# HiromasaYamanishi/furusato_recommend

Hardware: AMD Instinct MI355X
Metric: BPR positive-edges/sec (LightGCN-3 d=64, 1000000 x 100000 / 20000000 edges) (higher is better)
Workload: dtype f32; 1 GPU; C2: LightGCN 3-layer d=64, synthetic 1000000 users x 100000 items / 20000000 edges (uniform); users=1000000, items=100000, edges=20000000, graph=uniform, dim=64, layers=3, bpr_batch_per_rank=2048, global_batch=2048, ranks=1, parallelism=dp1 (user-sharded, RCCL none gradient exchange)

## Files before the change

furusato_recommend_amd/_lib.py:

```python
from __future__ import annotations

import ctypes
import os
from ctypes import (POINTER, Structure, c_float, c_int, c_int32, c_int64,
                    c_size_t, c_uint64, c_void_p, c_char_p)

import torch

_HERE = os.path.dirname(os.path.abspath(__file__))
LIB_PATH = os.environ.get("MIREC_LIB") or os.path.join(_HERE, "libmirec.so")

MIREC_OK = 0
ERR_WORKSPACE = 4
ERR_RANGE = 5
IN_PRESCALED, IN_RAW, IN_SPARSE, IN_NONE = 0, 1, 2, 3
SUPPORTED_DIMS = (4, 8, 16, 32, 64, 128, 256)


class MirecError(RuntimeError):
    pass


class CSR(Structure):
    _fields_ = [
        ("rowptr", c_void_p), ("col", c_void_p), ("dinv", c_void_p),
        ("n_rows", c_int64), ("nnz", c_int64), ("split", c_int32),
        ("_pad", c_int32), ("n_long", c_int64), ("n_seg", c_int64),
        ("long_rows", c_void_p), ("long_segptr", c_void_p),
        ("seg_row", c_void_p), ("seg_beg", c_void_p),
        ("col_sorted", c_void_p), ("n_sorted", c_int64), ("val", c_void_p),
    ]


class AdamH(Structure):
    _fields_ = [
        ("one_minus_beta1", c_float), ("beta2", c_float),
        ("one_minus_beta2", c_float), ("neg_step_size", c_float),
        ("bc2_sqrt", c_float), ("eps", c_float),
    ]


class Prop(Structure):
    _fields_ = [
        ("dim", c_int32), ("in_mode", c_int32), ("x_in", c_void_p),
        ("slot", c_void_p), ("seed_in", c_void_p), ("seed", c_void_p),
        ("addend", c_void_p), ("seed2", c_void_p), ("divisor", c_float),
        ("_pad", c_float), ("out", c_void_p), ("xs_out", c_void_p),
        ("param", c_void_p), ("exp_avg", c_void_p), ("exp_avg_sq", c_void_p),
        ("adam", AdamH), ("partial", c_void_p), ("row_mask", c_void_p),
        ("in_mask", c_void_p), ("out_mask", c_void_p), ("row_list", c_void_p),
        ("row_count", c_void_p),
        ("row_list_cap", c_int64), ("narrow_max", c_int32), ("adam_stream", c_int32),
        ("wide_list", c_void_p), ("wide_count", c_void_p),
        ("scale_src", c_void_p), ("scale_dst", c_void_p), ("scale_next", c_void_p),
    ]


class Drop(Structure):
    _fields_ = [("keep_prob", c_float), ("transposed", c_int32), ("seed", c_uint64)]


class SeedBits(Structure):
    _fields_ = [("bits", c_void_p), ("split", c_int64), ("shift", c_int32 * 2),
                ("words", c_int32 * 2)]


class Sweep(Structure):
    _fields_ = [
        ("row0", c_int64), ("n_rows", c_int64), ("n_src", c_int64),
        ("tile_rows", c_int32), ("group_rows", c_int32), ("groups", c_int32),
        ("n_tiles", c_int32), ("band_rows", c_int32), ("_pad", c_int32),
        ("gptr", c_void_p), ("ent", c_void_p),
    ]


class SweepWave(Structure):
    _fields_ = [
        ("row0", c_int64), ("n_rows", c_int64), ("src0", c_int64), ("n_src", c_int64),
        ("n_slots", c_int64),
        ("tile_rows", c_int32), ("wave_rows", c_int32), ("n_tiles", c_int32),
# ... 438 lines not shown
```

furusato_recommend_amd/csrc/prop.hip:

```cpp
#include <mutex>
#include <set>
#include <type_traits>
#include <utility>

#include "common.h"

namespace mirec {

struct PropK {
  const int64_t *rowptr;
  const int32_t *col;
  const float *dinv;
  int64_t n_rows;
  int64_t n_seg;
  const int32_t *seg_row;
  const int64_t *seg_beg;
  int32_t split;
  const float *x_in;
  const int32_t *slot;
  const float *seed_in;
  const float *seed;
  const float *addend;
  const float *seed2;
  float divisor;
// ... 106 lines not shown
          v[u] = f4_zero();
      }
#pragma unroll
      for (int u = 0; u < UNROLL; ++u) {
        if (MODE != MIREC_IN_PRESCALED || WEIGHTED)
          acc = f4_fma(w[u], v[u], acc);
        else
          acc = f4_add(acc, v[u]);
      }
    }
  }
  if constexpr (DROPOUT) acc = f4_scale(a.drop_scale, acc);
  return acc;
}

template <int D>
__device__ __forceinline__ float4 combine_groups(float4 s) {
  constexpr int LPR = D / 4;
#pragma unroll
  for (int m = LPR; m < 64; m <<= 1) s = f4_add(s, f4_shfl_xor(s, m));
  return s;
}

typedef float f32x4_t __attribute__((ext_vector_type(4)));
__device__ __forceinline__ float4 ld4_nt(const float *p) {
  const f32x4_t v = __builtin_nontemporal_load(reinterpret_cast<const f32x4_t *>(p));
  return make_float4(v.x, v.y, v.z, v.w);
}
__device__ __forceinline__ void st4_nt(float *p, float4 v) {
  const f32x4_t t = {v.x, v.y, v.z, v.w};
  __builtin_nontemporal_store(t, reinterpret_cast<f32x4_t *>(p));
}

template <int D, bool SCALED = false, bool STREAM = false>
__device__ __forceinline__ void row_epilogue(const PropK &a, int64_t row, float4 s, int sub) {
  const float di = a.dinv[row];
  float dn = di;
  if (SCALED && a.xs_out != nullptr) dn = a.scale_next[row];
  const int64_t off = row * D + sub * 4;
  float4 z = f4_scale(di, s);
  int sl = -1;
  if (a.slot != nullptr && (a.seed != nullptr || a.seed2 != nullptr)) sl = a.slot[row];
  if (a.seed != nullptr && sl >= 0) z = f4_add(z, ld4(a.seed + (int64_t)sl * D + sub * 4));
  if (a.xs_out != nullptr && a.param == nullptr) st4(a.xs_out + off, f4_scale(dn, z));
  if (a.out == nullptr && a.param == nullptr) return;
  if (a.out_mask != nullptr && a.param == nullptr && a.out_mask[row] == 0) return;
  float4 o = z;
  if (a.addend != nullptr) o = f4_add(o, ld4(a.addend + off));
  if (a.divisor != 1.f) o = f4_div(o, a.divisor);
  if (a.seed2 != nullptr && sl >= 0) o = f4_add(o, ld4(a.seed2 + (int64_t)sl * D + sub * 4));
  if (a.param != nullptr) {
    float4 p, m, v;
    if constexpr (STREAM) {
      p = ld4_nt(a.param + off), m = ld4_nt(a.m + off), v = ld4_nt(a.v + off);
    } else {
      p = ld4(a.param + off), m = ld4(a.m + off), v = ld4(a.v + off);
    }
    adam1(p.x, m.x, v.x, o.x, a.adam);
    adam1(p.y, m.y, v.y, o.y, a.adam);
    adam1(p.z, m.z, v.z, o.z, a.adam);
    adam1(p.w, m.w, v.w, o.w, a.adam);
    if constexpr (STREAM) {
      st4_nt(a.param + off, p);
      st4_nt(a.m + off, m);
      st4_nt(a.v + off, v);
    } else {
      st4(a.param + off, p);
      st4(a.m + off, m);
      st4(a.v + off, v);
    }
    if (a.out != nullptr) st4(a.out + off, o);
    if (a.xs_out != nullptr) st4(a.xs_out + off, f4_scale(dn, p));
  } else {
    st4(a.out + off, o);
  }
}

constexpr int kWavesPerBlock = 4;

template <int D, int UNROLL, int MODE, bool MASKED, bool ROWMASK, bool WEIGHTED, bool SCALED,
          bool DROPOUT, bool STREAM = false>
__device__ __forceinline__ void prop_work(const PropK &a, int64_t w, int64_t nrows,
                                          int64_t row_waves) {
  constexpr int LPR = D / 4;
  constexpr int G = 64 / LPR;
  constexpr int NARROW_UNROLL = UNROLL < 4 ? 4 : UNROLL;
  const int lane = threadIdx.x & 63;
  const int sub = lane % LPR;
  const int grp = lane / LPR;
  if (w < row_waves) {
    const int64_t idx = w * G + grp;
    bool have = idx < nrows;
    int32_t row = 0;
    if (have) row = (ROWMASK && a.row_list != nullptr) ? a.row_list[idx] : (int32_t)idx;
    if (ROWMASK && have) have = bit_set(a.row_mask, row);
    int64_t beg = 0, end = 0;
    if (have) {
      beg = a.rowptr[row];
      end = a.rowptr[row + 1];
      if (a.split > 0 && end - beg > a.split) {
        have = false;
        beg = end = 0;
      }
    }
    const int64_t deg = have ? end - beg : 0;
    if (G > 1 && __ballot(deg > a.narrow_max) == 0ull) {
      float4 s = gather<D, NARROW_UNROLL, MODE, MASKED, WEIGHTED, true, SCALED, DROPOUT>(
          a, beg, end, lane, row);
      if (have) row_epilogue<D, SCALED, STREAM>(a, row, s, sub);
// ... 437 lines not shown
  int32_t n_tiles;
  int32_t band_rows;
  int32_t n_bands;
  int32_t row_bits;
};

constexpr int kAuxNone = 0, kAuxPace = 1, kAuxStamp = 2;
constexpr int kPaceLabels = 8;
constexpr int kPaceLineWords = 32;
constexpr int kPaceRegionWords = (2 * kPaceLabels + 1) * kPaceLineWords;
constexpr int kPaceMaxNaps = 8;
constexpr int kPaceMaxNapUnits = 16;
constexpr int kXccIdReg = 20 | (3 << 11);

struct SweepAuxK {
  unsigned *ws;
  int32_t lead;
  int32_t every;
  int32_t nap;
  long long *stamps;
  int32_t *meta;
};

__device__ __forceinline__ unsigned pace_read(const unsigned *p) {
  unsigned v;
  asm volatile("s_load_dword %0, %1, 0x0 glc\n\ts_waitcnt lgkmcnt(0)"
               : "=&s"(v)
               : "s"(p)
               : "memory");
  return v;
}

template <int D, int U, bool SCALED, int AUX = kAuxNone, bool PACKED = false,
          bool STREAM = false, bool INMASK = false>
__device__ __forceinline__ void sweep_wave_work(const PropK &a, const SweepWaveK &s,
                                                const SweepAuxK &x = SweepAuxK{}) {
  constexpr int LPR = D / 4;
  constexpr int G = 64 / LPR;
  constexpr int NB = 64 / (U * G);
  static_assert(G == 4 && U * G == MIREC_SWEEP_BATCH && kSweepThreads / 64 == MIREC_SWEEP_WAVES,
                "the host layout's steps, batches and waves");
  static_assert(!INMASK || (!SCALED && !STREAM && AUX != kAuxStamp && NB >= 3),
                "the masked forms a step uses");
  extern __shared__ float4 sweep_acc[];
  const int lane = threadIdx.x & 63;
  const int sub = lane % LPR;
  const int g = lane / LPR;
  const int wid = __builtin_amdgcn_readfirstlane(threadIdx.x >> 6);
  using Slot = typename std::conditional<PACKED, unsigned, long long>::type;
  const Slot *slots = reinterpret_cast<const Slot *>(s.slot);
  [[maybe_unused]] const int col_bits = 32 - s.row_bits;
  const Slot kPadRow = PACKED ? (Slot)(~0u << col_bits) : (Slot)0xffffffff00000000ull;
  const int64_t last = s.n_slots - 1;
  [[maybe_unused]] auto slot_col = [&](Slot v) -> int64_t {
    if constexpr (PACKED) return s.src0 + (int64_t)(v & ~kPadRow);
    return (int64_t)(v & 0xffffffffll);
  };
  int adv = 0, told = 0, due = 0;
  unsigned *pace_reg = nullptr, *pace_sum = nullptr;
  if constexpr (AUX == kAuxPace) {
    const int label = (int)__builtin_amdgcn_s_getreg(kXccIdReg) & (kPaceLabels - 1);
    pace_reg = x.ws + (2 * label) * kPaceLineWords;
    pace_sum = pace_reg + kPaceLineWords;
    due = x.every;
    if (wid == 0 && lane == 0)
      (void)__hip_atomic_fetch_add(pace_reg, 1u, __ATOMIC_RELAXED, __HIP_MEMORY_SCOPE_AGENT);
  }
  auto pace = [&]() {
    if constexpr (AUX == kAuxPace) {
      if (wid != 0) return;
      ++adv;
      if (--due != 0) return;
      due = x.every;
      if (lane == 0)
        (void)__hip_atomic_fetch_add(pace_sum, (unsigned)(adv - told), __ATOMIC_RELAXED,
                                     __HIP_MEMORY_SCOPE_AGENT);
// ... 79 lines not shown
#pragma unroll
        for (int u = 0; u < U; ++u) {
          const int src = k * U * G + u * G + g;
          const int j = __shfl(lcol, src);
          r[u] = __shfl(crow, src);
          v[u] = ld4(a.x_in + (int64_t)j * D + sub * 4);
        }
#pragma unroll
        for (int u = 0; u < U; ++u) {
          if (pr[u] >= 0) {
            float4 *p = &sweep_acc[pr[u] * LPR + sub];
            *p = f4_add(*p, pv[u]);
          }
        }
#pragma unroll
        for (int u = 0; u < U; ++u) {
          pv[u] = v[u];
          pr[u] = r[u];
        }
      }
      pos += 64;
      cur = nxt;
      if constexpr (INMASK) {
        asm volatile("" : "+v"(nmask));
        cmask = nmask;
      }
    }
    while (band + 1 < s.n_bands) {
      pace();
      __builtin_amdgcn_s_barrier();
      ++band;
      stamp(band);
    }
#pragma unroll
    for (int u = 0; u < U; ++u) {
      if (pr[u] >= 0) {
        float4 *p = &sweep_acc[pr[u] * LPR + sub];
        *p = f4_add(*p, pv[u]);
      }
    }
    for (int lr = lr0 + g; lr < lr1; lr += G)
      row_epilogue<D, SCALED, STREAM>(a, s.row0 + tile_row0 + lr, sweep_acc[lr * LPR + sub],
                                      sub);
    if constexpr (AUX == kAuxStamp) {
      stamp(s.n_bands);
      if (wid == 0) {
        long long *o = x.stamps + (int64_t)tile * (s.n_bands + 1);
        for (int b = lane; b <= s.n_bands; b += 64) o[b] = stamp_lds[b];
        if (lane == 0) {
          x.meta[2 * tile] = (int32_t)blockIdx.x;
          x.meta[2 * tile + 1] = (int32_t)__builtin_amdgcn_s_getreg(kXccIdReg);
        }
      }
    }
    __syncthreads();
  }
  if constexpr (AUX == kAuxPace) {
    if (wid == 0 && lane == 0) {
      (void)__hip_atomic_fetch_add(pace_sum, 0u - (unsigned)told, __ATOMIC_RELAXED,
                                   __HIP_MEMORY_SCOPE_AGENT);
      (void)__hip_atomic_fetch_add(pace_reg, 0u - 1u, __ATOMIC_RELAXED, __HIP_MEMORY_SCOPE_AGENT);
      asm volatile("s_waitcnt vmcnt(0)" ::: "memory");
      unsigned *done = x.ws + 2 * kPaceLabels * kPaceLineWords;
      const unsigned left = __hip_atomic_fetch_add(done, 1u, __ATOMIC_RELAXED,
                                                   __HIP_MEMORY_SCOPE_AGENT);
      if (left == gridDim.x - 1) {
        for (int i = 0; i <= 2 * kPaceLabels; ++i)
          __hip_atomic_store(x.ws + i * kPaceLineWords, 0u, __ATOMIC_RELAXED,
                             __HIP_MEMORY_SCOPE_AGENT);
      }
    }
  }
}

template <int D, int U, bool SCALED, bool PACKED = false, bool STREAM = false>
__global__ __launch_bounds__(kSweepThreads) __attribute__((amdgpu_waves_per_eu(4, 4)))
MIREC_NO_PK_F32 void prop_sweep_wave_kernel(PropK a, SweepWaveK s) {
  sweep_wave_work<D, U, SCALED, kAuxNone, PACKED, STREAM>(a, s);
}

template <int D, int U, bool SCALED, int AUX, bool PACKED = false, bool STREAM = false>
__global__ __launch_bounds__(kSweepThreads) __attribute__((amdgpu_waves_per_eu(4, 4)))
MIREC_NO_PK_F32 void prop_sweep_wave_aux_kernel(PropK a, SweepWaveK s, SweepAuxK x) {
  sweep_wave_work<D, U, SCALED, AUX, PACKED, STREAM>(a, s, x);
}

template <int D, int U, bool PACKED>
__global__ __launch_bounds__(kSweepThreads) __attribute__((amdgpu_waves_per_eu(4, 4)))
MIREC_NO_PK_F32 void prop_sweep_wave_masked_kernel(PropK a, SweepWaveK s) {
  sweep_wave_work<D, U, false, kAuxNone, PACKED, false, true>(a, s);
}

template <int D, int U, int AUX, bool PACKED>
__global__ __launch_bounds__(kSweepThreads) __attribute__((amdgpu_waves_per_eu(4, 4)))
MIREC_NO_PK_F32 void prop_sweep_wave_masked_aux_kernel(PropK a, SweepWaveK s, SweepAuxK x) {
  sweep_wave_work<D, U, false, AUX, PACKED, false, true>(a, s, x);
}

using PropFn = void (*)(PropK);

template <int D, int UNROLL>
static PropFn prop_kernel_for(int mode, bool masked, bool rowmask, bool weighted, bool scaled,
                              bool dropout) {
  if (mode == MIREC_IN_SPARSE) masked = true;
  if (mode == MIREC_IN_NONE) weighted = dropout = false;
#define MIREC_PROP_CASE(MODE_W, MASKED)                               \
  case (MODE_W) * 2 + (MASKED):                                       \
    return rowmask ? prop_kernel<D, UNROLL, (MODE_W), MASKED, true>   \
                   : prop_kernel<D, UNROLL, (MODE_W), MASKED, false>;
  switch ((mode | (weighted ? kWeighted : 0) | (scaled ? kScaled : 0) |
           (dropout ? kDropout : 0)) * 2 + masked) {
    MIREC_PROP_CASE(MIREC_IN_PRESCALED | kWeighted, false)
    MIREC_PROP_CASE(MIREC_IN_PRESCALED, false)
    MIREC_PROP_CASE(MIREC_IN_PRESCALED | kWeighted, true)
    MIREC_PROP_CASE(MIREC_IN_PRESCALED, true)
    MIREC_PROP_CASE(MIREC_IN_RAW | kWeighted, false)
    MIREC_PROP_CASE(MIREC_IN_RAW, false)
    MIREC_PROP_CASE(MIREC_IN_RAW | kWeighted, true)
    MIREC_PROP_CASE(MIREC_IN_RAW, true)
    MIREC_PROP_CASE(MIREC_IN_SPARSE | kWeighted, true)
    MIREC_PROP_CASE(MIREC_IN_SPARSE, true)
    MIREC_PROP_CASE(MIREC_IN_PRESCALED | kScaled, false)
    MIREC_PROP_CASE(MIREC_IN_PRESCALED | kScaled, true)
    MIREC_PROP_CASE(MIREC_IN_RAW | kScaled, false)
    MIREC_PROP_CASE(MIREC_IN_RAW | kScaled, true)
    MIREC_PROP_CASE(MIREC_IN_SPARSE | kScaled, true)
    MIREC_PROP_CASE(MIREC_IN_NONE | kScaled, false)
    MIREC_PROP_CASE(MIREC_IN_PRESCALED | kDropout, false)
    MIREC_PROP_CASE(MIREC_IN_PRESCALED | kDropout, true)
// ... 246 lines not shown
  }
  return w->grid > 0 && w->grid <= w->n_tiles;
}

static int sweep_lds_allow(const void *kernel, size_t lds) {
  if (lds <= (size_t)kSweepLdsDefault) return MIREC_OK;
  static std::mutex mu;
  static std::set<std::pair<const void *, int>> raised;
  int dev = 0;
  MIREC_HIP(hipGetDevice(&dev));
  std::lock_guard<std::mutex> lock(mu);
  if (raised.count({kernel, dev}) != 0) return MIREC_OK;
  MIREC_HIP(hipFuncSetAttribute(kernel, hipFuncAttributeMaxDynamicSharedMemorySize,
                                kSweepLdsMax));
  raised.insert({kernel, dev});
  return MIREC_OK;
}

struct SweepStamp {
  const mirec_sweep_wave_t *layout;
  int64_t *stamps;
  int64_t stamps_len;
  int32_t *meta;
};

static int32_t sweep_wave_bands(const mirec_sweep_wave_t *w) {
  return (int32_t)std::max<int64_t>(1, (w->n_src + w->band_rows - 1) / w->band_rows);
}

template <int D>
static int launch_sweep_wave(const PropK &k, const mirec_sweep_wave_t *w, hipStream_t st,
                             const mirec_sweep_pace_t *pace = nullptr, int block = 0,
                             const SweepStamp *stamp = nullptr, bool stream = false,
                             bool masked = false) {
  SweepWaveK s;
  s.wptr = w->wptr;
  s.slot = reinterpret_cast<const long long *>(w->slot);
  s.n_slots = w->n_slots;
  s.row0 = w->row0;
  s.n_rows = w->n_rows;
  s.src0 = w->src0;
  s.tile_rows = w->tile_rows;
  s.wave_rows = w->wave_rows;
  s.n_tiles = w->n_tiles;
  s.band_rows = w->band_rows;
  s.n_bands = sweep_wave_bands(w);
  s.row_bits = w->row_bits;
  size_t lds = (size_t)w->tile_rows * D * sizeof(float);
  const bool scaled = k.scale_next != nullptr;
  const bool packed = w->row_bits != 0;
  stream = stream && packed && k.param != nullptr;
  if (masked && (scaled || stamp != nullptr || k.in_mask == nullptr))
    return MIREC_ERR_ARG;
  if (masked && pace != nullptr && pace->every[block] > 0) {
    SweepAuxK x = {};
    x.ws = reinterpret_cast<unsigned *>(pace->ws) + block * kPaceRegionWords;
    x.lead = pace->lead_bands[block];
    x.every = pace->every[block];
    x.nap = pace->nap[block];
    const auto kernel = packed ? prop_sweep_wave_masked_aux_kernel<D, 4, kAuxPace, true>
                               : prop_sweep_wave_masked_aux_kernel<D, 4, kAuxPace, false>;
    const int rc = sweep_lds_allow(reinterpret_cast<const void *>(kernel), lds);
    if (rc != MIREC_OK) return rc;
    hipLaunchKernelGGL(kernel, dim3((unsigned)w->grid), dim3(kSweepThreads), lds, st, k, s, x);
  } else if (masked) {
    const auto kernel = packed ? prop_sweep_wave_masked_kernel<D, 4, true>
                               : prop_sweep_wave_masked_kernel<D, 4, false>;
    const int rc = sweep_lds_allow(reinterpret_cast<const void *>(kernel), lds);
    if (rc != MIREC_OK) return rc;
    hipLaunchKernelGGL(kernel, dim3((unsigned)w->grid), dim3(kSweepThreads), lds, st, k, s);
  } else if (stamp != nullptr) {
    SweepAuxK x = {};
    x.stamps = reinterpret_cast<long long *>(stamp->stamps);
    x.meta = stamp->meta;
    lds += (size_t)(s.n_bands + 1) * sizeof(long long);
    if (packed) return MIREC_ERR_ARG;
    const auto kernel = scaled ? prop_sweep_wave_aux_kernel<D, 4, true, kAuxStamp>
                               : prop_sweep_wave_aux_kernel<D, 4, false, kAuxStamp>;
    if (lds > (size_t)kSweepLdsDefault &&
        hipFuncSetAttribute(reinterpret_cast<const void *>(kernel),
                            hipFuncAttributeMaxDynamicSharedMemorySize, (int)lds) != hipSuccess)
      return MIREC_ERR_HIP;
    hipLaunchKernelGGL(kernel, dim3((unsigned)w->grid), dim3(kSweepThreads), lds, st, k, s, x);
  } else if (pace != nullptr && pace->every[block] > 0) {
    SweepAuxK x = {};
    x.ws = reinterpret_cast<unsigned *>(pace->ws) + block * kPaceRegionWords;
    x.lead = pace->lead_bands[block];
// ... 93 lines not shown
  k.row_mask = p->row_mask;
  k.in_mask = p->in_mask;
  k.out_mask = p->out_mask;
  k.row_list = p->row_list;
  k.row_count = p->row_count;
  k.row_waves = 0;
  k.narrow_max = p->narrow_max;
  k.wide_list = p->wide_list;
  k.wide_count = p->wide_count;
  k.val = c->val;
  const bool scaled =
      p->scale_src != nullptr || p->scale_dst != nullptr || p->scale_next != nullptr;
  MIREC_CHECK_ARG(!scaled || c->val == nullptr);
  k.scale_src = k.scale_next = nullptr;
  if (scaled) {
    k.scale_src = p->scale_src != nullptr ? p->scale_src : c->dinv;
    k.dinv = p->scale_dst != nullptr ? p->scale_dst : c->dinv;
    k.scale_next = p->scale_next != nullptr ? p->scale_next : c->dinv;
  }
  const bool dropout = drop != nullptr && drop->keep_prob != 0.f;
  if (dropout) {
    uint32_t thresh_m1 = 0;
    MIREC_CHECK_ARG(edge_drop_thresh(drop->keep_prob, &thresh_m1));
    MIREC_CHECK_ARG(c->val == nullptr && !scaled);
    k.drop_key = edge_drop_key(drop->seed);
    k.drop_thresh_m1 = thresh_m1;
    k.drop_transposed = drop->transposed != 0;
    k.scale_next = nullptr;
    k.drop_scale = 1.f / drop->keep_prob;
  }
  const int64_t cap = p->row_list_cap;
  hipStream_t st = reinterpret_cast<hipStream_t>(stream);
  const bool nt = p->adam_stream != 0 && p->param != nullptr;
  if (stamp != nullptr) {
    const mirec_sweep_wave_t *w = stamp->layout;
    MIREC_CHECK_ARG(w != nullptr && stamp->stamps != nullptr && stamp->meta != nullptr);
    MIREC_CHECK_ARG(sweep_launch_qualifies(c, p) && w->row0 >= 0 && w->n_rows > 0 &&
                    w->row0 + w->n_rows <= c->n_rows &&
                    sweep_wave_valid(c, w, w->row0, w->n_rows));
    MIREC_CHECK_ARG(stamp->stamps_len >= (int64_t)w->n_tiles * (sweep_wave_bands(w) + 1));
    return launch_sweep_wave<64>(k, w, st, nullptr, 0, stamp);
  }
  if (sweep_qualifies(c, p, sw)) return launch_sweep<64, 4>(c, k, sw, st);
  if (wi != nullptr && sweep_launch_qualifies(c, p) &&
      sweep_wave_valid(c, wi, wi->row0, c->n_rows - wi->row0)) {
    const int rc = launch_sweep_wave<64>(k, wi, st, pace, 0, nullptr, nt);
    if (rc != MIREC_OK || wi->row0 == 0) return rc;
    if (sweep_wave_valid(c, wu, 0, wi->row0))
      return launch_sweep_wave<64>(k, wu, st, pace, 1, nullptr, nt);
    return launch_head<64, 4>(c, k, wi->row0, st);
  }
  if (masked_blocks != 0 && p->in_mask != nullptr && !scaled && wi != nullptr &&
      sweep_launch_qualifies(c, p, true) &&
      sweep_wave_valid(c, wi, wi->row0, c->n_rows - wi->row0)) {
    const bool mi = (masked_blocks & MIREC_SWEEP_MASKED_ITEMS) != 0;
    const bool mu = (masked_blocks & MIREC_SWEEP_MASKED_USERS) != 0 && wi->row0 > 0 &&
                    sweep_wave_valid(c, wu, 0, wi->row0);
    if (mi || mu) {
      const int rc = mi ? launch_sweep_wave<64>(k, wi, st, pace, 0, nullptr, false, true)
                        : launch_tail<64, 4>(c, k, wi->row0, st);
      if (rc != MIREC_OK || wi->row0 == 0) return rc;
      return mu ? launch_sweep_wave<64>(k, wu, st, pace, 1, nullptr, false, true)
                : launch_head<64, 4>(c, k, wi->row0, st);
    }
  }
  if (seeded != nullptr) {
    switch (p->dim) {
      case 4: return launch_seeded<4, 1>(k, seeded, c->nnz, cap, st);
      case 8: return launch_seeded<8, 1>(k, seeded, c->nnz, cap, st);
      case 16: return launch_seeded<16, 1>(k, seeded, c->nnz, cap, st);
      case 32: return launch_seeded<32, 2>(k, seeded, c->nnz, cap, st);
      case 64: return launch_seeded<64, 4>(k, seeded, c->nnz, cap, st);
      case 128: return launch_seeded<128, 4>(k, seeded, c->nnz, cap, st);
      case 256: return launch_seeded<256, 4>(k, seeded, c->nnz, cap, st);
    }
    return MIREC_ERR_DIM;
  }
  switch (p->dim) {
    case 4: return launch_prop<4, 1>(c, k, cap, p->in_mode, st, dropout);
    case 8: return launch_prop<8, 1>(c, k, cap, p->in_mode, st, dropout);
    case 16: return launch_prop<16, 1>(c, k, cap, p->in_mode, st, dropout);
    case 32: return launch_prop<32, 2>(c, k, cap, p->in_mode, st, dropout);
    case 64: return launch_prop<64, 4>(c, k, cap, p->in_mode, st, dropout, nt);
    case 128: return launch_prop<128, 4>(c, k, cap, p->in_mode, st, dropout);
    case 256: return launch_prop<256, 8>(c, k, cap, p->in_mode, st, dropout);
  }
  return MIREC_ERR_DIM;
}

}

extern "C" int mirec_propagate(const mirec_csr_t *c, const mirec_prop_t *p,
                               mirec_stream_t stream) {
  return mirec_propagate_sweep(c, p, nullptr, stream);
}
// ... 119 lines not shown
```

furusato_recommend_amd/engine.py:

```python
from __future__ import annotations

import ctypes
import math
import os

import torch

from . import _lib
from ._lib import (IN_NONE, IN_PRESCALED, IN_RAW, IN_SPARSE, Prop, adam_hparams,
                   check, lib, ptr)
from .graph import Graph

SWEEP_FORM = "wave"
SWEEP_USERS = True
LAYER_SUM_ROWS = "self"
SWEEP_PACE = {"items": (8, 16, 16), "users": (4, 4, 16)}
SEEDED_FIRST = True
ADAM_STREAM = True
SWEEP_INMASK = "items"
_INMASK_BLOCKS = {"off": 0, "items": 1, "users": 2, "both": 3}
SEEDED_LDS_BYTES = 16 * 1024


def seed_bit_layout(n0: int, n1: int, budget: int):
    def words(n, s):
        return -(-(-(-n // (1 << s))) // 32)

    def fit(n, share):
        s = 0
        while s < 31 and words(n, s) > 1 and 4 * words(n, s) > share:
            s += 1
        return s
    n = (int(n0), int(n1))
    small = 0 if n[0] <= n[1] else 1
    shift, w = [0, 0], [0, 0]
    shift[small] = fit(n[small], int(budget) * 7 // 8)
    w[small] = words(n[small], shift[small])
    shift[1 - small] = fit(n[1 - small], int(budget) - 4 * w[small])
    w[1 - small] = words(n[1 - small], shift[1 - small])
    w[1] += -(w[0] + w[1]) % 4
    return tuple(shift), tuple(w)


def prop_launch_bytes(in_mode: int, n_nodes: int, nnz: int, dim: int, *, slot=False,
                      xs_out=False, addend=False, out=False, adam=False, weighted=False,
                      scaled=False) -> int:
    N, D = n_nodes, dim
    row = N * D * 4
    b = (N + 1) * 8 + N * 4
    if in_mode == IN_PRESCALED:
        b += nnz * (D * 4 + 4)
    elif in_mode == IN_RAW:
        b += nnz * (D * 4 + 4 + 4)
# ... 183 lines not shown
        i32 = dict(dtype=torch.int32, device=dev)
        self.acc = torch.empty(N, D, **f32)
        self.x0s = torch.empty(N, D, **f32) if self.L > 0 else None
        self.xs = [torch.empty(N, D, **f32), torch.empty(N, D, **f32)] if self.L > 1 else \
            [torch.empty(N, D, **f32)] if self.L == 1 else []
        self.slot = torch.full((N,), -1, **i32)
        words = (N + 15) // 16 * 4
        nu = graph.n_users if graph.m_items > 0 else N
        self._bit_cap = (-(-nu // 32), -(-(N - nu) // 32))
        self._bm = torch.zeros(2 * words + (sum(self._bit_cap) + 3) // 4 * 4, **i32)
        self.bm_self, self.bm_hop = self._bm[:words], self._bm[words:2 * words]
        self._seed_bits_mem = self._bm[2 * words:]
        B3 = max((2 + self.n_neg) * self.max_batch, 2 * self.max_batch + self.n_shared)
        self.self_list = torch.zeros(B3, **i32)
        self.self_count = torch.zeros(1, **i32)
        self._self_cap = 0
        cap = N if self.prune else 1
        self.s_lists = (torch.zeros(cap, **i32), torch.zeros(cap, **i32))
        self.hop_lists = (torch.zeros(cap, **i32), torch.zeros(cap, **i32))
        self.list_counts = torch.zeros(4, **i32)
        self.use_hop_list = True
        self.reuse_prescaled = True
        self.layer_sum_rows = LAYER_SUM_ROWS
        self.use_sweep = True
        self._group_sizes = (None, None, None)
        self._wave_sizes = {"items": (None, None), "users": (None, None), "max_grid": None}
        self.sweep_wave = self.sweep_wave_users = None
        self._sweep_form, self._sweep_users = SWEEP_FORM, SWEEP_USERS
        self._sweep_packed = None
        self.adam_stream = ADAM_STREAM
        self.sweep_pace = SWEEP_PACE
        self._pace_ws = None
        self._sweep_inmask = SWEEP_INMASK
        self._wave_layouts()
        self.sparse_filter = "auto"
        self.seeded_first = SEEDED_FIRST
        self._seeded_lds_bytes = SEEDED_LDS_BYTES
        self._seed_bits = None
        self._bits_ready = False
        self._masks_ready = False
        self.narrow_max = 64
        self.seed_p = torch.empty(B3, D, **f32)
        self.seed_e = torch.empty(B3, D, **f32)
        self.coef = torch.empty(self.n_neg * self.max_batch, **f32)
        self.coef_pos = self.g_u = None
        self._shared = None
        self.softplus = torch.empty(self.max_batch, **f32)
        self.reg = torch.empty(self.max_batch, **f32)
        self.keys = torch.empty(B3, **i32)
        self.vals = torch.empty(B3, **i32)
        self.keys_sorted = torch.empty(B3, **i32)
        self.loss = torch.zeros(1, **f32)
        self.partial = graph.partial_buffer(D)
        self._ws = None
        self._ws_bytes = 0
        self._ensure_ws(self.max_batch)
        self.prop_events = None
        self._seeds = None
        self._merged = None
        self._x0s_token = None
        self._acc_full = None
        self.edge_dropout = None
        self._drop = None

    @staticmethod
    def dropout_seed(seed: int, step: int) -> int:
# ... 64 lines not shown
                p.scale_next = a if direction == "bwd_last" else b
            else:
                raise ValueError(f"direction: 'fwd', 'bwd' or 'bwd_last', got {direction!r}")
        p.dim = self.dim
        p.in_mode = in_mode
        p.x_in = ptr(x_in)
        p.slot = self.slot.data_ptr() if (seed_in is not None or seed is not None
                                          or seed2 is not None) else None
        p.seed_in = ptr(seed_in)
        p.seed = ptr(seed)
        p.addend = ptr(addend)
        p.seed2 = ptr(seed2)
        p.divisor = float(divisor)
        p.out = ptr(out)
        p.xs_out = ptr(xs_out)
        if adam is not None:
            state, hp = adam
            p.param = param.data_ptr()
            p.exp_avg = state.exp_avg.data_ptr()
            p.exp_avg_sq = state.exp_avg_sq.data_ptr()
            p.adam = hp
        part = g.partial_buffer(self.dim)
        p.partial = ptr(part)
        p.row_mask = ptr(row_mask)
        p.in_mask = ptr(in_mask)
        p.out_mask = ptr(out_mask)
        p.row_list = ptr(row_list)
        p.row_count = ptr(row_count)
        p.row_list_cap = int(row_list_cap)
        p.wide_list = ptr(wide_list)
        p.wide_count = ptr(wide_count)
        p.narrow_max = int(self.narrow_max)
        p.adam_stream = int(bool(self.adam_stream))
        ev = self.prop_events
        if ev is not None:
            s, e = torch.cuda.Event(enable_timing=True), torch.cuda.Event(enable_timing=True)
            s.record()
        on = self.use_sweep and g is self.g
        if stamp is not None:
            lay, stamps, meta = stamp
            check(lib.mirec_sweep_wave_stamp(g.csr_ptr(), ctypes.byref(p), lay.ptr(),
                                             stamps.data_ptr(), stamps.numel(), meta.data_ptr(),
                                             _lib.stream_handle()), "sweep_wave_stamp")
        elif self._drop is not None:
            if direction not in ("fwd", "bwd", "bwd_last"):
                raise ValueError(f"direction: 'fwd', 'bwd' or 'bwd_last', got {direction!r}")
            drop = _lib.Drop(keep_prob=self._drop[0], transposed=int(direction != "fwd"),
                             seed=self._drop[1])
            check(lib.mirec_propagate_drop(g.csr_ptr(), ctypes.byref(p), ctypes.byref(drop),
                                           _lib.stream_handle()), "propagate_drop")
        elif seeded:
            p.in_mask = None
            check(lib.mirec_propagate_seeded(g.csr_ptr(), ctypes.byref(p),
                                             ctypes.byref(self._seed_bits_struct()),
                                             _lib.stream_handle()), "propagate_seeded")
        elif on and self._sweep_form == "wave":
            wi, wu = self.sweep_wave, self.sweep_wave_users if self._sweep_users else None
            pace = self._pace_struct()
            args = (g.csr_ptr(), ctypes.byref(p), wi.ptr() if wi is not None else None,
                    wu.ptr() if wu is not None else None,
                    ctypes.byref(pace) if pace is not None else None)
            blocks = _INMASK_BLOCKS[self._sweep_inmask] if inmask_sweep else 0
            if blocks and in_mask is not None:
                check(lib.mirec_propagate_sweep_wave_masked(*args, blocks, _lib.stream_handle()),
                      "propagate")
            else:
# ... 751 lines not shown
```

include/mirec.h:

```cpp
#ifndef MIREC_H
#define MIREC_H

#include <stddef.h>
#include <stdint.h>

#ifdef __cplusplus
extern "C" {
#endif

#define MIREC_ABI_VERSION 1

enum mirec_status {
  MIREC_OK = 0,
  MIREC_ERR_ARG = 1,
  MIREC_ERR_DIM = 2,
  MIREC_ERR_HIP = 3,
  MIREC_ERR_WORKSPACE = 4,
  MIREC_ERR_RANGE = 5
};

typedef void *mirec_stream_t;

const char *mirec_strerror(int code);
int mirec_abi_version(void);
// ... 41 lines not shown
  const float *val;
} mirec_csr_t;

int mirec_csr_sort_rows(const int64_t *rowptr, const int32_t *col, int64_t n_rows,
                        int32_t *col_sorted);


enum mirec_in_mode {
  MIREC_IN_PRESCALED = 0,
  MIREC_IN_RAW = 1,
  MIREC_IN_SPARSE = 2,
  MIREC_IN_NONE = 3
};

typedef struct mirec_adam_hparams {
  float one_minus_beta1;
  float beta2;
  float one_minus_beta2;
  float neg_step_size;
  float bc2_sqrt;
  float eps;
} mirec_adam_hparams_t;

typedef struct mirec_prop {
  int32_t dim;
  int32_t in_mode;
  const float *x_in;
  const int32_t *slot;
  const float *seed_in;
  const float *seed;
  const float *addend;
  const float *seed2;
  float divisor;
  float _pad;
  float *out;
  float *xs_out;
  float *param;
  float *exp_avg;
  float *exp_avg_sq;
  mirec_adam_hparams_t adam;
  float *partial;
  const uint8_t *row_mask;
  const uint8_t *in_mask;
  const uint8_t *out_mask;
  const int32_t *row_list;
  const int32_t *row_count;
  int64_t row_list_cap;
  int32_t narrow_max;
  int32_t adam_stream;
  const int32_t *wide_list;
  const int32_t *wide_count;
  const float *scale_src;
  const float *scale_dst;
  const float *scale_next;
} mirec_prop_t;

int mirec_propagate(const mirec_csr_t *csr, const mirec_prop_t *p,
                    mirec_stream_t stream);

int mirec_edge_keep_mask(const int64_t *rowptr, const int32_t *col, int64_t n_rows,
                         uint64_t seed, float keep_prob, int32_t transposed,
                         uint8_t *keep);


typedef struct mirec_drop {
  float keep_prob;
  int32_t transposed;
// ... 682 lines not shown
```

Baseline: 623,100 positive-edges/s.

## Pipeline sweep tile epilogue with prefetched Adam and addend loads

After: 626,700 positive-edges/s (median of 6 runs). Within noise of the previous version (+0.6%).

```diff
diff --git a/furusato_recommend_amd/_lib.py b/furusato_recommend_amd/_lib.py
--- a/furusato_recommend_amd/_lib.py
+++ b/furusato_recommend_amd/_lib.py
@@ -45,7 +45,7 @@
         ("dim", c_int32), ("in_mode", c_int32), ("x_in", c_void_p),
         ("slot", c_void_p), ("seed_in", c_void_p), ("seed", c_void_p),
         ("addend", c_void_p), ("seed2", c_void_p), ("divisor", c_float),
-        ("_pad", c_float), ("out", c_void_p), ("xs_out", c_void_p),
+        ("sweep_epilogue", c_int32), ("out", c_void_p), ("xs_out", c_void_p),
         ("param", c_void_p), ("exp_avg", c_void_p), ("exp_avg_sq", c_void_p),
         ("adam", AdamH), ("partial", c_void_p), ("row_mask", c_void_p),
         ("in_mask", c_void_p), ("out_mask", c_void_p), ("row_list", c_void_p),
diff --git a/furusato_recommend_amd/csrc/prop.hip b/furusato_recommend_amd/csrc/prop.hip
--- a/furusato_recommend_amd/csrc/prop.hip
+++ b/furusato_recommend_amd/csrc/prop.hip
@@ -162,26 +162,52 @@
   __builtin_nontemporal_store(t, reinterpret_cast<f32x4_t *>(p));
 }
 
-template <int D, bool SCALED = false, bool STREAM = false>
-__device__ __forceinline__ void row_epilogue(const PropK &a, int64_t row, float4 s, int sub) {
-  const float di = a.dinv[row];
+struct EpiInline {
+  static constexpr bool kAhead = false;
+};
+
+template <int D, bool SCALED, bool STREAM, class In>
+__device__ __forceinline__ void epilogue_body(const PropK &a, int64_t row, float4 s, int sub,
+                                              const In &in) {
+  float di;
+  if constexpr (In::kAhead)
+    di = in.di;
+  else
+    di = a.dinv[row];
   float dn = di;
-  if (SCALED && a.xs_out != nullptr) dn = a.scale_next[row];
+  if constexpr (!In::kAhead) {
+    if (SCALED && a.xs_out != nullptr) dn = a.scale_next[row];
+  }
   const int64_t off = row * D + sub * 4;
   float4 z = f4_scale(di, s);
   int sl = -1;
-  if (a.slot != nullptr && (a.seed != nullptr || a.seed2 != nullptr)) sl = a.slot[row];
+  if constexpr (In::kAhead) {
+    sl = in.sl;
+  } else {
+    if (a.slot != nullptr && (a.seed != nullptr || a.seed2 != nullptr)) sl = a.slot[row];
+  }
   if (a.seed != nullptr && sl >= 0) z = f4_add(z, ld4(a.seed + (int64_t)sl * D + sub * 4));
   if (a.xs_out != nullptr && a.param == nullptr) st4(a.xs_out + off, f4_scale(dn, z));
   if (a.out == nullptr && a.param == nullptr) return;
-  if (a.out_mask != nullptr && a.param == nullptr && a.out_mask[row] == 0) return;
+  if constexpr (In::kAhead) {
+    if (in.om == 0) return;
+  } else {
+    if (a.out_mask != nullptr && a.param == nullptr && a.out_mask[row] == 0) return;
+  }
   float4 o = z;
-  if (a.addend != nullptr) o = f4_add(o, ld4(a.addend + off));
+  if (a.addend != nullptr) {
+    if constexpr (In::kAhead)
+      o = f4_add(o, in.addend(a, off));
+    else
+      o = f4_add(o, ld4(a.addend + off));
+  }
   if (a.divisor != 1.f) o = f4_div(o, a.divisor);
   if (a.seed2 != nullptr && sl >= 0) o = f4_add(o, ld4(a.seed2 + (int64_t)sl * D + sub * 4));
   if (a.param != nullptr) {
     float4 p, m, v;
-    if constexpr (STREAM) {
+    if constexpr (In::kAhead) {
+      p = in.t.p, m = in.t.m, v = in.t.v;
+    } else if constexpr (STREAM) {
       p = ld4_nt(a.param + off), m = ld4_nt(a.m + off), v = ld4_nt(a.v + off);
     } else {
       p = ld4(a.param + off), m = ld4(a.m + off), v = ld4(a.v + off);
@@ -205,6 +231,116 @@
     st4(a.out + off, o);
   }
 }
+
+template <int D, bool SCALED = false, bool STREAM = false>
+__device__ __forceinline__ void row_epilogue(const PropK &a, int64_t row, float4 s, int sub) {
+  epilogue_body<D, SCALED, STREAM>(a, row, s, sub, EpiInline{});
+}
+
+constexpr int kEpiNone = 0, kEpiAdam = 1, kEpiAddend = 2;
+
+template <int D, bool STREAM>
+struct TileEpilogue {
+  static constexpr int LPR = D / 4, G = 64 / LPR;
+  struct Streams {
+    float4 p, m, v;
+  };
+  template <int KIND>
+  struct Ahead {
+    static constexpr bool kAhead = true;
+    float di;
+    int sl;
+    int om;
+    const Streams &t;
+    __device__ __forceinline__ float4 addend(const PropK &a, int64_t off) const {
+      if constexpr (KIND == kEpiAddend) return t.p;
+      return ld4(a.addend + off);
+    }
+  };
+  int64_t row_base;
+  int n, g, sub, kind;
+  float di;
+  int sl, om;
+  Streams s0;
+
+  template <int KIND>
+  __device__ __forceinline__ void issue(const PropK &a, int k, Streams &t) const {
+    [[maybe_unused]] const int64_t off = (row_base + min(k, n - 1)) * D + sub * 4;
+    if constexpr (KIND == kEpiAdam) {
+      if constexpr (STREAM) {
+        t.p = ld4_nt(a.param + off), t.m = ld4_nt(a.m + off), t.v = ld4_nt(a.v + off);
+      } else {
+        t.p = ld4(a.param + off), t.m = ld4(a.m + off), t.v = ld4(a.v + off);
+      }
+    }
+    if constexpr (KIND == kEpiAddend) t.p = ld4(a.addend + off);
+  }
+
+  __device__ __forceinline__ void begin(const PropK &a, int64_t base, int rows, int lane) {
+    row_base = base, n = rows, g = lane / LPR, sub = lane % LPR;
+    s0.p = s0.m = s0.v = f4_zero();
+    di = 0.f, sl = -1, om = 1;
+    kind = kEpiNone;
+    if (a.param != nullptr)
+      kind = kEpiAdam;
+    else if (a.addend != nullptr && a.out != nullptr && a.out_mask == nullptr)
+      kind = kEpiAddend;
+    if (n <= 0) return;
+    const int64_t r = row_base + min(lane, n - 1);
+    di = a.dinv[r];
+    if (a.slot != nullptr && (a.seed != nullptr || a.seed2 != nullptr)) sl = a.slot[r];
+    if (a.out_mask != nullptr && a.param == nullptr) om = a.out_mask[r];
+    if (kind == kEpiAdam) issue<kEpiAdam>(a, g, s0);
+    if (kind == kEpiAddend) issue<kEpiAddend>(a, g, s0);
+  }
+
+  template <int KIND>
+  __device__ __forceinline__ void step(const PropK &a, const float4 *acc, int k0,
+                                       const Streams &t) const {
+    const int k = k0 + g;
+    const int kc = min(k, n - 1);
+    const float rdi = __int_as_float(__builtin_amdgcn_ds_bpermute(kc << 2, __float_as_int(di)));
+    const int rsl = __builtin_amdgcn_ds_bpermute(kc << 2, sl);
+    const int rom = __builtin_amdgcn_ds_bpermute(kc << 2, om);
+    const float4 s = acc[kc * LPR + sub];
+    if (k < n) {
+      const int64_t row = row_base + k;
+      __builtin_assume((a.param != nullptr) == (KIND == kEpiAdam));
+      const Ahead<KIND> in = {rdi, rsl, rom, t};
+      epilogue_body<D, false, STREAM>(a, row, s, sub, in);
+    }
+  }
+
+  template <int KIND>
+  __device__ __forceinline__ void run_kind(const PropK &a, const float4 *acc) {
+    Streams s1;
+    s1.p = s1.m = s1.v = f4_zero();
+    int k0 = 0;
+    while (k0 + G < n) {
+      issue<KIND>(a, k0 + G + g, s1);
+      step<KIND>(a, acc, k0, s0);
+      k0 += G;
+      if (k0 + G >= n) {
+        step<KIND>(a, acc, k0, s1);
+        return;
+      }
+      issue<KIND>(a, k0 + G + g, s0);
+      step<KIND>(a, acc, k0, s1);
+      k0 += G;
+    }
+    step<KIND>(a, acc, k0, s0);
+  }
+
+  __device__ __forceinline__ void run(const PropK &a, const float4 *acc) {
+    if (n <= 0) return;
+    if (kind == kEpiAdam)
+      run_kind<kEpiAdam>(a, acc);
+    else if (kind == kEpiAddend)
+      run_kind<kEpiAddend>(a, acc);
+    else
+      run_kind<kEpiNone>(a, acc);
+  }
+};
 
 constexpr int kWavesPerBlock = 4;
 
@@ -708,7 +844,7 @@
 }
 
 template <int D, int U, bool SCALED, int AUX = kAuxNone, bool PACKED = false,
-          bool STREAM = false, bool INMASK = false>
+          bool STREAM = false, bool INMASK = false, bool EPI = false>
 __device__ __forceinline__ void sweep_wave_work(const PropK &a, const SweepWaveK &s,
                                                 const SweepAuxK &x = SweepAuxK{}) {
   constexpr int LPR = D / 4;
@@ -718,6 +854,8 @@
                 "the host layout's steps, batches and waves");
   static_assert(!INMASK || (!SCALED && !STREAM && AUX != kAuxStamp && NB >= 3),
                 "the masked forms a step uses");
+  static_assert(!EPI || (!SCALED && PACKED && AUX != kAuxStamp),
+                "the forms with a pipelined tile epilogue");
   extern __shared__ float4 sweep_acc[];
   const int lane = threadIdx.x & 63;
   const int sub = lane % LPR;
@@ -863,6 +1001,8 @@
       ++band;
       stamp(band);
     }
+    [[maybe_unused]] TileEpilogue<D, STREAM> epi;
+    if constexpr (EPI) epi.begin(a, s.row0 + tile_row0 + lr0, lr1 - lr0, lane);
 #pragma unroll
     for (int u = 0; u < U; ++u) {
       if (pr[u] >= 0) {
@@ -870,9 +1010,13 @@
         *p = f4_add(*p, pv[u]);
       }
     }
-    for (int lr = lr0 + g; lr < lr1; lr += G)
-      row_epilogue<D, SCALED, STREAM>(a, s.row0 + tile_row0 + lr, sweep_acc[lr * LPR + sub],
-                                      sub);
+    if constexpr (EPI) {
+      epi.run(a, sweep_acc + lr0 * LPR);
+    } else {
+      for (int lr = lr0 + g; lr < lr1; lr += G)
+        row_epilogue<D, SCALED, STREAM>(a, s.row0 + tile_row0 + lr, sweep_acc[lr * LPR + sub],
+                                        sub);
+    }
     if constexpr (AUX == kAuxStamp) {
       stamp(s.n_bands);
       if (wid == 0) {
@@ -926,6 +1070,12 @@
 __global__ __launch_bounds__(kSweepThreads) __attribute__((amdgpu_waves_per_eu(4, 4)))
 MIREC_NO_PK_F32 void prop_sweep_wave_masked_aux_kernel(PropK a, SweepWaveK s, SweepAuxK x) {
   sweep_wave_work<D, U, false, AUX, PACKED, false, true>(a, s, x);
+}
+
+template <int D, int U, int AUX, bool STREAM, bool INMASK>
+__global__ __launch_bounds__(kSweepThreads) __attribute__((amdgpu_waves_per_eu(4, 4)))
+MIREC_NO_PK_F32 void prop_sweep_wave_epi_kernel(PropK a, SweepWaveK s, SweepAuxK x) {
+  sweep_wave_work<D, U, false, AUX, true, STREAM, INMASK, true>(a, s, x);
 }
 
 using PropFn = void (*)(PropK);
@@ -1238,7 +1388,7 @@
 static int launch_sweep_wave(const PropK &k, const mirec_sweep_wave_t *w, hipStream_t st,
                              const mirec_sweep_pace_t *pace = nullptr, int block = 0,
                              const SweepStamp *stamp = nullptr, bool stream = false,
-                             bool masked = false) {
+                             bool masked = false, bool epi = false) {
   SweepWaveK s;
   s.wptr = w->wptr;
   s.slot = reinterpret_cast<const long long *>(w->slot);
@@ -1258,7 +1408,27 @@
   stream = stream && packed && k.param != nullptr;
   if (masked && (scaled || stamp != nullptr || k.in_mask == nullptr))
     return MIREC_ERR_ARG;
-  if (masked && pace != nullptr && pace->every[block] > 0) {
+  if (epi && packed && !scaled && stamp == nullptr && w->wave_rows <= 64) {
+    SweepAuxK x = {};
+    const bool paced = pace != nullptr && pace->every[block] > 0;
+    if (paced) {
+      x.ws = reinterpret_cast<unsigned *>(pace->ws) + block * kPaceRegionWords;
+      x.lead = pace->lead_bands[block];
+      x.every = pace->every[block];
+      x.nap = pace->nap[block];
+    }
+    auto kernel = paced ? prop_sweep_wave_epi_kernel<D, 4, kAuxPace, false, false>
+                        : prop_sweep_wave_epi_kernel<D, 4, kAuxNone, false, false>;
+    if (masked)
+      kernel = paced ? prop_sweep_wave_epi_kernel<D, 4, kAuxPace, false, true>
+                     : prop_sweep_wave_epi_kernel<D, 4, kAuxNone, false, true>;
+    else if (stream)
+      kernel = paced ? prop_sweep_wave_epi_kernel<D, 4, kAuxPace, true, false>
+                     : prop_sweep_wave_epi_kernel<D, 4, kAuxNone, true, false>;
+    const int rc = sweep_lds_allow(reinterpret_cast<const void *>(kernel), lds);
+    if (rc != MIREC_OK) return rc;
+    hipLaunchKernelGGL(kernel, dim3((unsigned)w->grid), dim3(kSweepThreads), lds, st, k, s, x);
+  } else if (masked && pace != nullptr && pace->every[block] > 0) {
     SweepAuxK x = {};
     x.ws = reinterpret_cast<unsigned *>(pace->ws) + block * kPaceRegionWords;
     x.lead = pace->lead_bands[block];
@@ -1418,6 +1588,7 @@
   const int64_t cap = p->row_list_cap;
   hipStream_t st = reinterpret_cast<hipStream_t>(stream);
   const bool nt = p->adam_stream != 0 && p->param != nullptr;
+  const bool epi = p->sweep_epilogue != 0;
   if (stamp != nullptr) {
     const mirec_sweep_wave_t *w = stamp->layout;
     MIREC_CHECK_ARG(w != nullptr && stamp->stamps != nullptr && stamp->meta != nullptr);
@@ -1430,10 +1601,10 @@
   if (sweep_qualifies(c, p, sw)) return launch_sweep<64, 4>(c, k, sw, st);
   if (wi != nullptr && sweep_launch_qualifies(c, p) &&
       sweep_wave_valid(c, wi, wi->row0, c->n_rows - wi->row0)) {
-    const int rc = launch_sweep_wave<64>(k, wi, st, pace, 0, nullptr, nt);
+    const int rc = launch_sweep_wave<64>(k, wi, st, pace, 0, nullptr, nt, false, epi);
     if (rc != MIREC_OK || wi->row0 == 0) return rc;
     if (sweep_wave_valid(c, wu, 0, wi->row0))
-      return launch_sweep_wave<64>(k, wu, st, pace, 1, nullptr, nt);
+      return launch_sweep_wave<64>(k, wu, st, pace, 1, nullptr, nt, false, epi);
     return launch_head<64, 4>(c, k, wi->row0, st);
   }
   if (masked_blocks != 0 && p->in_mask != nullptr && !scaled && wi != nullptr &&
@@ -1443,10 +1614,10 @@
     const bool mu = (masked_blocks & MIREC_SWEEP_MASKED_USERS) != 0 && wi->row0 > 0 &&
                     sweep_wave_valid(c, wu, 0, wi->row0);
     if (mi || mu) {
-      const int rc = mi ? launch_sweep_wave<64>(k, wi, st, pace, 0, nullptr, false, true)
+      const int rc = mi ? launch_sweep_wave<64>(k, wi, st, pace, 0, nullptr, false, true, epi)
                         : launch_tail<64, 4>(c, k, wi->row0, st);
       if (rc != MIREC_OK || wi->row0 == 0) return rc;
-      return mu ? launch_sweep_wave<64>(k, wu, st, pace, 1, nullptr, false, true)
+      return mu ? launch_sweep_wave<64>(k, wu, st, pace, 1, nullptr, false, true, epi)
                 : launch_head<64, 4>(c, k, wi->row0, st);
     }
   }
diff --git a/furusato_recommend_amd/engine.py b/furusato_recommend_amd/engine.py
--- a/furusato_recommend_amd/engine.py
+++ b/furusato_recommend_amd/engine.py
@@ -19,6 +19,8 @@
 ADAM_STREAM = True
 SWEEP_INMASK = "items"
 _INMASK_BLOCKS = {"off": 0, "items": 1, "users": 2, "both": 3}
+SWEEP_EPILOGUE = "pipelined"
+_EPILOGUES = {"inline": 0, "pipelined": 1}
 SEEDED_LDS_BYTES = 16 * 1024
 
 
@@ -268,6 +270,7 @@
         self.sweep_pace = SWEEP_PACE
         self._pace_ws = None
         self._sweep_inmask = SWEEP_INMASK
+        self.sweep_epilogue = SWEEP_EPILOGUE
         self._wave_layouts()
         self.sparse_filter = "auto"
         self.seeded_first = SEEDED_FIRST
@@ -398,6 +401,10 @@
         p.wide_count = ptr(wide_count)
         p.narrow_max = int(self.narrow_max)
         p.adam_stream = int(bool(self.adam_stream))
+        if self.sweep_epilogue not in _EPILOGUES:
+            raise ValueError("sweep_epilogue: 'inline' or 'pipelined', "
+                             f"got {self.sweep_epilogue!r}")
+        p.sweep_epilogue = _EPILOGUES[self.sweep_epilogue]
         ev = self.prop_events
         if ev is not None:
             s, e = torch.cuda.Event(enable_timing=True), torch.cuda.Event(enable_timing=True)
diff --git a/include/mirec.h b/include/mirec.h
--- a/include/mirec.h
+++ b/include/mirec.h
@@ -97,7 +97,7 @@
   const float *addend;
   const float *seed2;
   float divisor;
-  float _pad;
+  int32_t sweep_epilogue;
   float *out;
   float *xs_out;
   float *param;
```
